# deflect-ca/banjax

Hardware: AMD Instinct MI355X
Metric: log lines/sec matched+rate-limited (node) at 1k rules; HBM GB/s vs peak (higher is better)
Workload: dtype u8

## Files before the change

banjax_amd/csrc/bjx_common.h:

```cpp
#pragma once
#include <stdint.h>

#ifdef __HIPCC__
#define BJX_HD __host__ __device__ __forceinline__
#define BJX_HDN __host__ __device__ inline
#else
#define BJX_HD inline
#define BJX_HDN inline
#endif

namespace bjx {


BJX_HD int32_t decode_rune_hd(const uint8_t *s, uint64_t n, int *width) {
  uint8_t b0 = s[0];
  if (b0 < 0x80) { *width = 1; return b0; }
  int need; uint8_t lo = 0x80, hi = 0xBF; int32_t r;
  if (b0 >= 0xC2 && b0 <= 0xDF) { need = 1; r = b0 & 0x1F; }
  else if (b0 == 0xE0) { need = 2; lo = 0xA0; r = b0 & 0x0F; }
  else if ((b0 >= 0xE1 && b0 <= 0xEC) || b0 == 0xEE || b0 == 0xEF) { need = 2; r = b0 & 0x0F; }
  else if (b0 == 0xED) { need = 2; hi = 0x9F; r = b0 & 0x0F; }
  else if (b0 == 0xF0) { need = 3; lo = 0x90; r = b0 & 0x07; }
  else if (b0 >= 0xF1 && b0 <= 0xF3) { need = 3; r = b0 & 0x07; }
  else if (b0 == 0xF4) { need = 3; hi = 0x8F; r = b0 & 0x07; }
  else { *width = 1; return 0xFFFD; }
  if (n < (uint64_t)need + 1 || s[1] < lo || s[1] > hi) { *width = 1; return 0xFFFD; }
  r = (r << 6) | (s[1] & 0x3F);
  for (int k = 2; k <= need; ++k) {
    if (s[k] < 0x80 || s[k] > 0xBF) { *width = 1; return 0xFFFD; }
    r = (r << 6) | (s[k] & 0x3F);
  }
  *width = need + 1;
  return r;
}


BJX_HD uint64_t mix64(uint64_t x) {
  x ^= x >> 33; x *= 0xff51afd7ed558ccdULL;
  x ^= x >> 33; x *= 0xc4ceb9fe1a85ec53ULL;
  x ^= x >> 33;
  return x;
}
inline uint32_t ld4(const uint8_t *p) {
  uint32_t v;
  __builtin_memcpy(&v, p, 4);
  return v;
}
#ifdef __HIPCC__
__device__ __forceinline__ uint32_t ld4(const uint8_t *p) {
  const uint32_t sh = (uint32_t)(reinterpret_cast<uintptr_t>(p) & 3);
  const uint32_t *w = reinterpret_cast<const uint32_t *>(p - sh);
  return sh ? __builtin_amdgcn_alignbyte(w[1], w[0], sh) : w[0];
}
#endif

BJX_HD uint32_t rotl32(uint32_t x, int r) { return (x << r) | (x >> (32 - r)); }

BJX_HD uint64_t hash_finish(uint32_t a, uint32_t b, uint32_t t);

BJX_HD uint64_t hash_bytes(const uint8_t *p, uint32_t n) {
  uint32_t a = 0x9E3779B9u ^ n, b = 0x7F4A7C15u + n * 0x85EBCA6Bu;
  uint32_t i = 0;
  for (; i + 4 <= n; i += 4) {
    const uint32_t w = ld4(p + i);
    a = rotl32(a ^ w, 7) * 0x27D4EB2Du;
    b = rotl32(b + w, 13) * 0x165667B1u;
  }
  uint32_t t = 0;
  for (uint32_t k = 0; i + k < n; ++k) t |= (uint32_t)p[i + k] << (8 * k);
  return hash_finish(a, b, t);
}

BJX_HD uint32_t host_fold_word(uint32_t w, uint32_t k) {
  const uint32_t r = (7u * k + 3u) & 31u;
  return (w << r) | (w >> ((32u - r) & 31u));
}
BJX_HD uint32_t host_fold_finish(uint32_t a, uint32_t n) {
  a ^= n * 0x9E3779B9u;
  a ^= a >> 15; a *= 0x2C1B3C6Du; a ^= a >> 12; a *= 0x297A2D39u; a ^= a >> 15;
  return a | 1u;
}
BJX_HD uint32_t host_fold(const uint8_t *p, uint32_t n) {
  uint32_t a = 0, k = 0, i = 0;
  for (; i + 4 <= n; i += 4, ++k) a ^= host_fold_word(ld4(p + i), k);
  if (i < n) {
    uint32_t t = 0;
    for (uint32_t b = 0; i + b < n; ++b) t |= (uint32_t)p[i + b] << (8 * b);
    a ^= host_fold_word(t, k);
  }
  return host_fold_finish(a, n);
}

BJX_HD uint64_t hash_finish(uint32_t a, uint32_t b, uint32_t t) {
  a = rotl32(a ^ t ^ 0xA5A5A5A5u, 7) * 0x27D4EB2Du;
  b = rotl32(b + t, 13) * 0x165667B1u;
  a ^= b >> 16; a *= 0x85EBCA6Bu; a ^= a >> 13; a *= 0xC2B2AE35u; a ^= a >> 16;
  b ^= a >> 15; b *= 0x2C1B3C6Du; b ^= b >> 12; b *= 0x297A2D39u; b ^= b >> 15;
  uint64_t h = ((uint64_t)a << 32) | b;
  if (h == 0 || h == ~0ULL) h = 0x1234567ULL;
  return h;
}


BJX_HD uint64_t search_stride(uint64_t lo, uint64_t hi, uint32_t K) { return (hi - lo + K - 1) / K; }
BJX_HD void search_narrow(uint64_t &lo, uint64_t &hi, uint64_t stride, uint32_t f, uint32_t K) {
  if (f == 0) { hi = lo; return; }
  uint64_t last = f - 1;
  if (f < K) hi = lo + (uint64_t)f * stride;
  else {
    last = (hi - 1 - lo) / stride;
    if (last > K - 1) last = K - 1;
  }
  lo += last * stride + 1;
}


BJX_HD int64_t go_sub(int64_t t, int64_t u) {
  int64_t d = (int64_t)((uint64_t)t - (uint64_t)u);
  if (((t ^ u) & (t ^ d)) < 0) return t < u ? INT64_MIN : INT64_MAX;
  return d;
}


BJX_HD bool window_past(int64_t ts, int64_t t0, int64_t interval) { return go_sub(ts, t0) > interval; }

BJX_HD bool window_step(int64_t ts, int64_t interval, int64_t limit, bool &valid, int64_t &hits, int64_t &start, uint32_t &mt) {
  if (!valid) { hits = 1; start = ts; mt = 0; valid = true; }
  else if (window_past(ts, start, interval)) { mt = 1; hits = 1; start = ts; }
  else { mt = 2; ++hits; }
  const bool ex = hits > limit;
  if (ex) hits = 0;
  return ex;
}

BJX_HD int64_t mod_pos(int64_t a, int64_t b) {
  if ((((uint64_t)a | (uint64_t)b) >> 32) == 0) return (int64_t)((uint32_t)a % (uint32_t)b);
  return a % b;
}

BJX_HD int64_t window_hits(int64_t h0, int64_t e, int64_t limit) {
  if (limit < 0) return 0;
  if (limit == INT64_MAX) return h0 + e;
  if (h0 > limit) return mod_pos(e - 1, limit + 1);
  return mod_pos(h0 + e, limit + 1);
}

BJX_HD int64_t ns_from_seconds(double f) {
  double x = f * 1e9;
  if (!(x >= -9223372036854775808.0 && x < 9223372036854775808.0)) return INT64_MIN;
  return (int64_t)x;
}


BJX_HD int lower_c(int c) { return (c >= 'A' && c <= 'Z') ? c + 32 : c; }

BJX_HD int parse_float_fast(const uint8_t *s, uint32_t n, double *out) {
  if (n == 0 || n > 40) return 1;
  uint64_t m = 0;
  int frac = -1, digits = 0;
  for (uint32_t i = 0; i < n; ++i) {
    uint8_t c = s[i];
    if (c >= '0' && c <= '9') {
      if (m != 0 || c != '0') ++digits;
      if (digits > 16) return 1;
      m = m * 10 + (c - '0');
      if (frac >= 0) ++frac;
    } else if (c == '.' && frac < 0) {
      frac = 0;
    } else {
      return 1;
    }
  }
  if (frac < 0) frac = 0;
  if (s[0] == '.' || (n == 1 && s[0] == '.')) return 1;
  if (m >= (1ULL << 53) || frac > 22) return 1;
  double p = 1.0;
  if (frac & 1) p *= 1e1;
  if (frac & 2) p *= 1e2;
  if (frac & 4) p *= 1e4;
  if (frac & 8) p *= 1e8;
  if (frac & 16) p *= 1e16;
  double f = (double)m;
  *out = frac ? f / p : f;
  return 0;
}

struct Decimal {
  uint8_t d[800];
  int nd, dp;
  bool neg, trunc;
};

BJX_HDN void dec_trim(Decimal *a) {
  while (a->nd > 0 && a->d[a->nd - 1] == 0) a->nd--;
  if (a->nd == 0) a->dp = 0;
}
BJX_HDN void dec_lshift(Decimal *a, unsigned k) {
  uint8_t tmp[824];
  int tw = 824;
  uint64_t n = 0;
  for (int r = a->nd - 1; r >= 0; --r) {
    n += (uint64_t)a->d[r] << k;
    uint64_t q = n / 10;
    tmp[--tw] = (uint8_t)(n - 10 * q);
    n = q;
  }
  while (n > 0) {
    uint64_t q = n / 10;
    tmp[--tw] = (uint8_t)(n - 10 * q);
    n = q;
  }
  int newnd = 824 - tw;
  int keep = newnd > 800 ? 800 : newnd;
  for (int i = 0; i < keep; ++i) a->d[i] = tmp[tw + i];
  for (int i = keep; i < newnd; ++i)
    if (tmp[tw + i]) a->trunc = true;
  a->dp += newnd - a->nd;
  a->nd = keep;
  dec_trim(a);
}
BJX_HDN void dec_rshift(Decimal *a, unsigned k) {
  int r = 0, w = 0;
  uint64_t n = 0;
  for (; (n >> k) == 0; ++r) {
    if (r >= a->nd) {
      if (n == 0) { a->nd = 0; return; }
      while ((n >> k) == 0) { n *= 10; ++r; }
      break;
    }
    n = n * 10 + a->d[r];
  }
  a->dp -= r - 1;
  const uint64_t mask = (1ULL << k) - 1;
  for (; r < a->nd; ++r) {
    uint64_t dig = n >> k;
    n &= mask;
    a->d[w++] = (uint8_t)dig;
    n = n * 10 + a->d[r];
  }
  while (n > 0) {
    uint64_t dig = n >> k;
    n &= mask;
    if (w < 800) a->d[w++] = (uint8_t)dig;
    else if (dig > 0) a->trunc = true;
    n = n * 10;
  }
  a->nd = w;
  dec_trim(a);
}
BJX_HDN void dec_shift(Decimal *a, int k) {
  if (a->nd == 0) return;
  if (k > 0) { while (k > 60) { dec_lshift(a, 60); k -= 60; } dec_lshift(a, (unsigned)k); }
  else if (k < 0) { while (k < -60) { dec_rshift(a, 60); k += 60; } dec_rshift(a, (unsigned)-k); }
}
BJX_HDN bool dec_round_up(const Decimal *a, int nd) {
  if (a->d[nd] == 5 && nd + 1 == a->nd) {
    if (a->trunc) return true;
    return nd > 0 && (a->d[nd - 1] % 2) != 0;
  }
  return a->d[nd] >= 5;
}
BJX_HDN uint64_t dec_rounded_integer(const Decimal *a) {
  if (a->dp > 20) return ~0ULL;
  int i = 0;
  uint64_t n = 0;
  for (; i < a->dp && i < a->nd; ++i) n = n * 10 + a->d[i];
  for (; i < a->dp; ++i) n *= 10;
  if (a->dp >= 0 && a->dp < a->nd && dec_round_up(a, a->dp)) ++n;
  return n;
}
BJX_HDN uint64_t dec_float_bits(Decimal *a, bool *overflow) {
  const int mantbits = 52, expbits = 11, bias = -1023;
  const int powtab[9] = {1, 3, 6, 9, 13, 16, 19, 23, 26};
  int exp = 0;
  uint64_t mant = 0;
  *overflow = false;
  if (a->nd == 0) { mant = 0; exp = bias; goto out; }
  if (a->dp > 310) goto ovf;
  if (a->dp < -330) { mant = 0; exp = bias; goto out; }
  while (a->dp > 0) {
    int n = a->dp >= 9 ? 27 : powtab[a->dp];
    dec_shift(a, -n);
    exp += n;
  }
  while (a->dp < 0 || (a->dp == 0 && a->d[0] < 5)) {
    int n = -a->dp >= 9 ? 27 : powtab[-a->dp];
    dec_shift(a, n);
    exp -= n;
  }
  exp--;
  if (exp < bias + 1) {
    int n = bias + 1 - exp;
    dec_shift(a, -n);
    exp += n;
  }
  if (exp - bias >= (1 << expbits) - 1) goto ovf;
  dec_shift(a, 1 + mantbits);
  mant = dec_rounded_integer(a);
// ... 280 lines not shown
```

banjax_amd/csrc/engine.hip:

```cpp
#include <hip/hip_runtime.h>
#include <hipcub/hipcub.hpp>

#include <algorithm>
#include <array>
#include <atomic>
#include <cstdio>
#include <cstdlib>
#include <cstring>
#include <map>
#include <tuple>
#include <memory>
#include <mutex>
#include <stdexcept>
#include <string>
#include <unordered_map>
#include <thread>
#include <vector>

#include "../../include/banjax_gpu.h"
#include "bjx_common.h"
#include "engine_types.h"
#include "regex_compiler.h"
#include "bans.h"

// ... 3072 lines not shown
      continue;
    }
    R v = s_rec[b];
    for (uint32_t u = b; u < e; ++u) {
      R nx;
      if (u + 1 < e) nx = s_rec[u + 1];
      s_out[u] = apply_step(v, tbase, rules, pr, interval, limit, valid, hits, start);
      v = nx;
    }
    st[q].hits = hits;
    st[q].start = start;
    st[q].valid = 1;
  }
  __syncthreads();
  const uint32_t s_lo = nh ? s_head[0] : n, s_hi = nh && s_cont ? s_head[nh - 1] : n;
  for (uint32_t i = s_lo + tid; i < s_hi; i += kBlock) {
    out_sorted[u0 + i] = s_out[i];
    if (wcnt) atomicAdd(&wcnt[u0 + i], 1u);
  }
}

constexpr int kBucketBits = 16;
constexpr uint32_t kBucketItems = 16;
constexpr uint32_t kBucketCap = kBlock * kBucketItems;
constexpr uint32_t kWaveRun = 8;

__global__ __launch_bounds__(kBlock) void k_bucket_bounds(uint64_t n_ev, const uint32_t *__restrict__ key, uint32_t L,
                                                          uint32_t nb, uint32_t *__restrict__ bstart) {
  const uint64_t i0 = ((uint64_t)blockIdx.x * blockDim.x + threadIdx.x) * 4;
  uint32_t k[4] = {0, 0, 0, 0};
  if (i0 + 4 <= n_ev) {
    const uint4 v = *reinterpret_cast<const uint4 *>(key + i0);
    k[0] = v.x; k[1] = v.y; k[2] = v.z; k[3] = v.w;
  } else {
    for (uint32_t j = 0; j < 4; ++j)
      if (i0 + j < n_ev) k[j] = key[i0 + j];
  }
  uint32_t prev = __shfl_up(k[3], 1);
  if ((threadIdx.x & 63) == 0 && i0 && i0 <= n_ev) prev = key[i0 - 1];
#pragma unroll
  for (uint32_t j = 0; j < 4; ++j) {
    const uint64_t i = i0 + j;
    if (i > n_ev) return;
    const uint32_t b = i < n_ev ? k[j] >> L : nb;
    const uint32_t lo = i ? (prev >> L) + 1 : 0u;
    for (uint32_t x = lo; x <= b; ++x) bstart[x] = (uint32_t)i;
    prev = k[j];
  }
}


template <typename R>
__device__ __forceinline__ void wave_chunk(uint32_t u0, uint32_t p, const R &rv, uint32_t na, bool first, int64_t tbase,
                                           const DevRule *__restrict__ rules, uint32_t &r0, int64_t &I, int64_t &Lim,
                                           bool &valid, int64_t &hits, int64_t &start, uint8_t *s_out,
                                           uint32_t *__restrict__ wcnt) {
  const uint32_t lane = threadIdx.x & 63;
  const bool act = lane < na;
  const uint32_t r = rv.rule_id();
  const int64_t ts = rv.time(tbase);
  if (first) {
    r0 = __shfl(r, 0);
    I = rules[r0].interval_ns;
    Lim = rules[r0].hits;
  }
  bool same = true;
  if (r != r0) same = rules[r].interval_ns == I && rules[r].hits == Lim;
  uint32_t mt = BJX_INSIDE_INTERVAL;
  bool ex = false;
  if (__ballot(!same) == 0) {
    int32_t a = valid ? -1 : 0;
    int64_t Tw = valid ? start : __shfl(ts, 0);
    uint32_t wa = 0, wmt = valid ? BJX_INSIDE_INTERVAL : BJX_FIRST_TIME;
    int64_t wh0 = valid ? hits : 0;
    for (;;) {
      const unsigned long long m = __ballot(act && (int32_t)lane > a && window_past(ts, Tw, I));
      if (!m) break;
      a = __ffsll(m) - 1;
      Tw = __shfl(ts, a);
      if ((int32_t)lane >= a) { wa = (uint32_t)a; wh0 = 0; wmt = BJX_OUTSIDE_INTERVAL; }
    }
    const int64_t hh = window_hits(wh0, (int64_t)(lane - wa) + 1, Lim);
    ex = hh == 0;
    if (lane == wa) mt = wmt;
    hits = __shfl(hh, (int)na - 1);
    start = Tw;
    valid = true;
  } else {
    uint32_t pr = 0xFFFFFFFFu;
    int64_t iv = 0, lm = 0;
    for (uint32_t i = 0; i < na; ++i) {
      const uint8_t o = apply_event(__shfl(r, (int)i), true, __shfl(ts, (int)i), rules, pr, iv, lm, valid, hits, start);
      if (lane == i) { mt = (o >> 1) & 3u; ex = (o & 8) != 0; }
    }
  }
  if (act) {
    s_out[p] = outcome_byte(rv.seen(), mt, ex);
    if (wcnt) atomicAdd(&wcnt[u0 + p], 1u);
  }
}

template <typename R>
__device__ __forceinline__ void bucket_wave_runs(const R *__restrict__ rec, uint32_t u0, uint32_t n, uint32_t nh, uint32_t nwv,
                                                 const uint16_t *s_ord_top, const uint16_t *s_head, const uint16_t *s_lk,
                                                 const uint16_t *s_perm, uint8_t *s_out, uint32_t qb, int64_t tbase,
                                                 const DevRule *__restrict__ rules, StSlot *__restrict__ st,
                                                 uint32_t *__restrict__ wcnt) {
  const uint32_t lane = threadIdx.x & 63;
  uint32_t t = threadIdx.x >> 6;
  if (t >= nwv) return;
  uint32_t b, e, q;
  auto run_at = [&](uint32_t tt, uint32_t &bb, uint32_t &ee, uint32_t &qq) {
    const uint32_t h = *(s_ord_top - tt);
    bb = s_head[h];
    ee = h + 1 < nh ? s_head[h + 1] : n;
    qq = qb | s_lk[bb];
  };
  auto pos_at = [&](uint32_t cc, uint32_t ee) { return (uint32_t)s_perm[cc + (lane < ee - cc ? lane : 0u)]; };
  run_at(t, b, e, q);
  uint32_t c = b;
  StSlot nslot = st[q];
  uint32_t np = pos_at(c, e);
  R nrv = rec[u0 + np];
  bool valid = false;
  int64_t hits = 0, start = 0, I = 0, Lim = 0;
  uint32_t r0 = 0;
  for (;;) {
    const uint32_t p = np, na = min(64u, e - c);
    const R rv = nrv;
    const bool first = c == b, last = c + 64 >= e;
    if (first) { valid = nslot.valid != 0; hits = nslot.hits; start = nslot.start; }
    uint32_t t2 = t, b2 = b, e2 = e, q2 = q, c2 = c + 64;
    if (last) {
      t2 = t + kBlock / 64;
      if (t2 < nwv) { run_at(t2, b2, e2, q2); c2 = b2; }
    }
    const bool more = t2 < nwv;
    if (more) {
      if (last) nslot = st[q2];
      np = pos_at(c2, e2);
      nrv = rec[u0 + np];
    }
    wave_chunk(u0, p, rv, na, first, tbase, rules, r0, I, Lim, valid, hits, start, s_out, wcnt);
    if (last && lane == 0) {
      st[q].hits = hits;
      st[q].start = start;
      st[q].valid = 1;
    }
    if (!more) break;
    t = t2; b = b2; e = e2; q = q2; c = c2;
  }
}

#ifdef BJX_BK_STOP
#define BJX_BK_STAGE(k)                                                           \
  if (BJX_BK_STOP == (k)) {                                                       \
    for (uint32_t i = tid; i < n; i += kBlock) out_sorted[u0 + i] = s_out[i];     \
    return;                                                                       \
  }
#define BJX_BK_LANE_RUNS (BJX_BK_STOP == 3 ? nfront : nh - nwv)
#else
#define BJX_BK_STAGE(k)
#define BJX_BK_LANE_RUNS (nh - nwv)
#endif
#ifdef BJX_BK_CENSUS
__device__ unsigned long long g_bk_census[8];
#endif

template <typename R>
__global__ __launch_bounds__(kBlock) void k_bucket_apply(const uint32_t *__restrict__ key, const R *__restrict__ rec,
                                                         const uint32_t *__restrict__ bstart, uint32_t L, int64_t tbase,
                                                         const DevRule *__restrict__ rules, StSlot *__restrict__ st,
                                                         uint8_t *__restrict__ out_sorted, uint32_t *__restrict__ big,
                                                         unsigned long long *__restrict__ n_big, uint32_t *__restrict__ wcnt,
                                                         uint32_t wave_min) {
  using Sort = hipcub::BlockRadixSort<uint32_t, kBlock, kBucketItems>;
  static_assert(kBucketCap <= 4096, "positions ride in 12 key bits");
  constexpr uint32_t kLongRun = 8;
  __shared__ union {
    typename Sort::TempStorage sort;
    uint32_t lk[kBucketCap];
    uint16_t ho[2 * kBucketCap];
  } s_u;
  __shared__ uint16_t s_lk[kBucketCap];
  __shared__ uint16_t s_perm[kBucketCap];
  uint16_t *const s_head = s_u.ho;
  uint16_t *const s_ord = s_u.ho + kBucketCap;
  __shared__ uint8_t s_out[kBucketCap];
  __shared__ uint32_t s_wsum[kBlock / 64], s_front, s_back, s_nwave;
  const uint32_t tid = threadIdx.x, lane = tid & 63, wave = tid >> 6;
  const uint32_t bk = blockIdx.x, u0 = bstart[bk], n = bstart[bk + 1] - u0;
  if (n == 0) return;
  if (n > kBucketCap) {
    if (tid == 0) big[atomicAdd(n_big, 1ull)] = bk;
    return;
  }
  const uint32_t mask = (1u << L) - 1u;
  for (uint32_t i = tid; i < n; i += kBlock) s_u.lk[i] = key[u0 + i] & mask;
#ifdef BJX_BK_STOP
  for (uint32_t i = tid; i < n; i += kBlock) s_out[i] = outcome_byte(true, BJX_INSIDE_INTERVAL, false);
#endif
  if (tid == 0) { s_front = 0; s_back = 0; s_nwave = 0; }
  __syncthreads();
  uint32_t k[kBucketItems];
#pragma unroll
  for (uint32_t j = 0; j < kBucketItems; ++j) {
    const uint32_t i = tid * kBucketItems + j;
    k[j] = ((i < n ? s_u.lk[i] : mask) << 12) | i;
  }
  __syncthreads();
  Sort(s_u.sort).SortBlockedToStriped(k, 12, 12 + (int)L);
  __syncthreads();
#pragma unroll
  for (uint32_t j = 0; j < kBucketItems; ++j) {
    const uint32_t r = j * kBlock + tid;
    s_lk[r] = (uint16_t)(k[j] >> 12);
    s_perm[r] = (uint16_t)(k[j] & 0xFFFu);
  }
  __syncthreads();
  BJX_BK_STAGE(1)
  uint32_t fl = 0;
#pragma unroll
  for (uint32_t j = 0; j < kBucketItems; ++j) {
    const uint32_t i = tid * kBucketItems + j;
    if (i < n && (i == 0 || s_lk[i] != s_lk[i - 1])) fl |= 1u << j;
  }
  const uint32_t cnt = __popc(fl);
  uint32_t x = cnt;
#pragma unroll
  for (int d = 1; d < 64; d <<= 1) {
    const uint32_t y = __shfl_up(x, d);
    if (lane >= (uint32_t)d) x += y;
  }
  if (lane == 63) s_wsum[wave] = x;
  __syncthreads();
  uint32_t base = x - cnt, nh = 0;
  for (uint32_t w = 0; w < kBlock / 64; ++w) {
    if (w < wave) base += s_wsum[w];
    nh += s_wsum[w];
  }
  for (uint32_t j = 0; fl; ++j, fl >>= 1)
    if (fl & 1) s_head[base++] = (uint16_t)(tid * kBucketItems + j);
  __syncthreads();
  for (uint32_t h = tid; h < nh; h += kBlock) {
    const uint32_t len = (h + 1 < nh ? s_head[h + 1] : n) - s_head[h];
    if (len >= wave_min) s_ord[kBucketCap - 1 - atomicAdd(&s_nwave, 1u)] = (uint16_t)h;
    else if (len >= kLongRun) s_ord[atomicAdd(&s_front, 1u)] = (uint16_t)h;
    else s_ord[nh - 1 - atomicAdd(&s_back, 1u)] = (uint16_t)h;
#ifdef BJX_BK_CENSUS
    atomicAdd(&g_bk_census[0], (unsigned long long)len);
    atomicAdd(&g_bk_census[1], 1ull);
    for (uint32_t c = 0; c < 3; ++c)
      if (len >= (8u << c * (c + 1) / 2)) {
        atomicAdd(&g_bk_census[2 + 2 * c], (unsigned long long)len);
        atomicAdd(&g_bk_census[3 + 2 * c], 1ull);
      }
#endif
  }
  __syncthreads();
  BJX_BK_STAGE(2)
  const uint32_t qb = bk << L;
  const uint32_t nwv = s_nwave, nfront = s_front;
  bucket_wave_runs(rec, u0, n, nh, nwv, s_ord + kBucketCap - 1, s_head, s_lk, s_perm, s_out, qb, tbase, rules, st, wcnt);
  for (uint32_t t = tid; t < BJX_BK_LANE_RUNS; t += kBlock) {
    const uint32_t h = s_ord[t < nfront ? t : t + nwv];
    const uint32_t b = s_head[h], e = h + 1 < nh ? s_head[h + 1] : n;
    const uint32_t q = qb | s_lk[b];
    const StSlot cur = st[q];
    bool valid = cur.valid != 0;
    int64_t hits = cur.hits, start = cur.start, interval = 0, limit = 0;
    uint32_t pr = 0xFFFFFFFFu;
    uint32_t p = s_perm[b];
    R rv = rec[u0 + p];
    for (uint32_t u = b; u < e; ++u) {
      R nx;
      uint32_t pn = 0;
      if (u + 1 < e) { pn = s_perm[u + 1]; nx = rec[u0 + pn]; }
      s_out[p] = apply_step(rv, tbase, rules, pr, interval, limit, valid, hits, start);
      if (wcnt) atomicAdd(&wcnt[u0 + p], 1u);
      rv = nx;
      p = pn;
    }
    st[q].hits = hits;
    st[q].start = start;
    st[q].valid = 1;
  }
  __syncthreads();
  for (uint32_t i = tid; i < n; i += kBlock) out_sorted[u0 + i] = s_out[i];
}

__global__ __launch_bounds__(kBlock) void k_big_gather(const uint4 *__restrict__ seg, uint32_t n_seg, uint64_t total,
                                                       const uint32_t *__restrict__ key, uint32_t *__restrict__ ko,
                                                       uint32_t *__restrict__ po) {
  const uint64_t i = (uint64_t)blockIdx.x * blockDim.x + threadIdx.x;
  if (i >= total) return;
  uint32_t lo = 0, hi = n_seg - 1;
  while (lo < hi) {
    const uint32_t mid = (lo + hi + 1) >> 1;
    if (seg[mid].z <= i) lo = mid;
    else hi = mid - 1;
  }
  const uint4 s = seg[lo];
  const uint32_t src = s.x + (uint32_t)(i - s.z);
  ko[i] = key[src];
  po[i] = src;
}

template <typename R>
__global__ __launch_bounds__(kBlock) void k_big_recs(uint64_t n, const uint32_t *__restrict__ pos, const R *__restrict__ rec,
                                                     R *__restrict__ out) {
  const uint64_t i = (uint64_t)blockIdx.x * blockDim.x + threadIdx.x;
  if (i < n) out[i] = rec[pos[i]];
}

__global__ __launch_bounds__(kBlock) void k_big_outs(uint64_t n, const uint32_t *__restrict__ pos, const uint8_t *__restrict__ o,
                                                     uint8_t *__restrict__ out_sorted, const uint32_t *__restrict__ wsrc,
                                                     uint32_t *__restrict__ wcnt) {
  const uint64_t i = (uint64_t)blockIdx.x * blockDim.x + threadIdx.x;
  if (i >= n) return;
  out_sorted[pos[i]] = o[i];
  if (wcnt) atomicAdd(&wcnt[pos[i]], wsrc[i]);
}

__device__ __forceinline__ uint32_t block_min_u32(uint32_t v, uint32_t *s_red) {
  for (int o = 32; o > 0; o >>= 1) v = min(v, (uint32_t)__shfl_xor((int)v, o));
  __syncthreads();
  if ((threadIdx.x & 63) == 0) s_red[threadIdx.x >> 6] = v;
  __syncthreads();
  uint32_t m = s_red[0];
  for (uint32_t w = 1; w < kBlock / 64; ++w) m = min(m, s_red[w]);
  return m;
}

template <typename P>
__device__ uint64_t block_first(uint64_t lo, uint64_t hi, P pred, uint32_t *s_red) {
  while (lo < hi) {
    const uint64_t stride = search_stride(lo, hi, kBlock);
    const uint64_t p = lo + (uint64_t)threadIdx.x * stride;
    const bool ok = p < hi && pred(p);
    const uint32_t f = block_min_u32(ok ? threadIdx.x : (uint32_t)kBlock, s_red);
    search_narrow(lo, hi, stride, f, kBlock);
  }
  return hi;
}

constexpr uint64_t kLongSerial = 512;

struct LongRuns {
  const uint64_t *head;
  uint64_t *end;
  uint64_t *off;
  int64_t *t0;
  int64_t *h0;
  uint32_t *flags;
  uint64_t *win;
  uint32_t *nwin;
  uint64_t n;
  uint32_t *wcnt;
};

template <typename Rec>
__global__ __launch_bounds__(kBlock) void k_long_ends(uint64_t n_ev, const uint32_t *__restrict__ key,
                                                      const Rec *__restrict__ rec, int64_t base, const StSlot *__restrict__ st,
                                                      const DevRule *__restrict__ rules, LongRuns R, uint64_t *__restrict__ len) {
  __shared__ uint32_t s_red[kBlock / 64];
  const uint64_t r = blockIdx.x;
  const uint64_t head = R.head[r];
  const uint32_t q = key[head];
  const uint64_t end = block_first(head + 1, n_ev, [&](uint64_t i) { return key[i] != q; }, s_red);
  if (threadIdx.x != 0) return;
  R.end[r] = end;
  len[r] = end - head;
// ... 4355 lines not shown
    if (kept_ips > n_ips || kept_bytes > used || kept_st > e->st_cap)
      throw BjxError(BJX_ERR_DEVICE, "internal: expiry counts exceed the tables");

    const uint64_t ip_cap = std::min(e->ip_cap, std::max(e->ip_cap0, next_pow2(kept_ips * 4 / 3 + 1024)));
    const uint64_t st_cap = std::min(e->st_cap, std::max(e->st_cap0, next_pow2(kept_st * 4 / 3 + 1024)));
    const uint64_t arena_cap = std::min(S.arena_cap, std::max(e->arena_cap0, next_pow2(2 * kept_bytes + 4096)));
    ExpAlloc nw;
    IpSlot *n_ip = nw.get<IpSlot>(ip_cap);
    uint32_t *n_first = nw.get<uint32_t>(ip_cap);
    uint64_t *n_off = nw.get<uint64_t>(ip_cap);
    uint32_t *n_len = nw.get<uint32_t>(ip_cap);
    uint32_t *n_ipst = nw.get<uint32_t>(ip_cap);
    uint8_t *n_arena = nw.get<uint8_t>(arena_cap);
    StSlot *n_stt = nw.get<StSlot>(st_cap);
    if (nw.nomem) throw BjxError(BJX_ERR_NOMEM, "bjx_state_expire: no device memory for the new tables (state unchanged)");
    HIP_OK(hipEventRecord(ev[2], st));
    HIP_OK(hipMemsetAsync(n_ip, 0, ip_cap * sizeof(IpSlot), st));
    HIP_OK(hipMemsetAsync(n_first, 0xFF, ip_cap * 4, st));
    HIP_OK(hipMemsetAsync(n_ipst, 0xFF, ip_cap * 4, st));
    HIP_OK(hipMemsetAsync(n_stt, 0, st_cap * sizeof(StSlot), st));
    if (n_ips) {
      hipLaunchKernelGGL(k_exp_arena, dim3(grid_for(n_ips)), dim3(kBlock), 0, st, n_ips, keep, nid, noff, S.ip_off, S.ip_len,
                         S.arena, used, n_arena, arena_cap, n_off, n_len);
      HIP_OK(hipGetLastError());
    }
    hipLaunchKernelGGL(k_exp_st, dim3(grid_for(e->st_cap)), dim3(kBlock), 0, st, e->st_cap, S.st, cutoff_ns, n_ips, nid, n_stt,
                       st_cap - 1);
    HIP_OK(hipGetLastError());
    hipLaunchKernelGGL(k_exp_ip, dim3(grid_for(e->ip_cap)), dim3(kBlock), 0, st, e->ip_cap, S.ip, n_ips, keep, nid, n_ip,
                       ip_cap - 1);
    HIP_OK(hipGetLastError());
    HIP_OK(hipEventRecord(ev[3], st));
    HIP_OK(hipStreamSynchronize(st));

    nw.take();
    for (void *p : {(void *)S.ip, (void *)S.ip_first, (void *)S.ip_off, (void *)S.ip_len, (void *)S.ip_st, (void *)S.arena,
                    (void *)S.st})
      (void)hipFree(p);
    S.ip = n_ip; S.ip_first = n_first; S.ip_off = n_off; S.ip_len = n_len; S.ip_st = n_ipst; S.arena = n_arena; S.st = n_stt;
    S.ip_mask = ip_cap - 1;
    S.st_mask = st_cap - 1;
    S.arena_cap = arena_cap;
    S.ip_st_cap = ip_cap;
    if (st_cap > (1ull << 32)) S.hot_name = kNone;
    else if (e->st_cap > (1ull << 32)) e->bound_uid = 0;
    e->ip_cap = ip_cap;
    e->st_cap = st_cap;
    e->sort2_hold = 0;
    hipLaunchKernelGGL(k_exp_counters, dim3(1), dim3(64), 0, st, S.counters, kept_ips, kept_bytes, (uint64_t)kept_st);
    HIP_OK(hipGetLastError());
    HIP_OK(hipStreamSynchronize(st));
    e->host_counters[0] = kept_ips; e->host_counters[1] = kept_bytes; e->host_counters[2] = kept_st;
    e->counters_fresh = false;
    if (out) {
      float a = 0, b = 0;
      HIP_OK(hipEventElapsedTime(&a, ev[0], ev[1]));
      HIP_OK(hipEventElapsedTime(&b, ev[2], ev[3]));
      out->states_before = n_st; out->states_dropped = n_st - std::min<uint64_t>(n_st, kept_st);
      out->ips_before = n_ips; out->ips_dropped = n_ips - kept_ips;
      out->arena_bytes_before = used; out->arena_bytes_after = kept_bytes;
      out->device_bytes_before = bytes_before;
      out->device_bytes_after = state_device_bytes(ip_cap, st_cap, arena_cap);
      out->device_ms = (double)a + (double)b;
    }
    return BJX_OK;
  } catch (const BjxError &x) {
    e->last_error = x.what();
    return x.code;
  } catch (const std::bad_alloc &) {
    e->last_error = "host out of memory";
    return BJX_ERR_NOMEM;
  }
}

extern "C" size_t bjx_state_dump(bjx_engine *e, char *out, size_t cap) {
  if (!e) return 0;
  std::lock_guard<std::mutex> g(e->mu);
  try {
    HIP_OK(hipSetDevice(e->device));
    read_counters(e);
    const uint64_t n_ips = e->host_counters[0], used = e->host_counters[1];
    std::vector<uint64_t> off(n_ips);
    std::vector<uint32_t> len(n_ips);
    std::vector<StSlot> st(e->st_cap);
    std::vector<uint8_t> arena(used);
    HIP_OK(hipMemcpy(off.data(), e->S.ip_off, n_ips * 8, hipMemcpyDeviceToHost));
    HIP_OK(hipMemcpy(len.data(), e->S.ip_len, n_ips * 4, hipMemcpyDeviceToHost));
    HIP_OK(hipMemcpy(arena.data(), e->S.arena, used, hipMemcpyDeviceToHost));
    HIP_OK(hipMemcpy(st.data(), e->S.st, e->st_cap * sizeof(StSlot), hipMemcpyDeviceToHost));
    std::vector<std::vector<std::pair<uint32_t, uint64_t>>> per_ip(n_ips);
    for (uint64_t i = 0; i < e->st_cap; ++i)
      if (st[i].key && st[i].valid) per_ip[(st[i].key >> 24) - 1].push_back({(uint32_t)(st[i].key & 0xFFFFFF), i});
    std::string s;
    char buf[96];
    for (uint64_t id = 0; id < n_ips; ++id) {
      s.append(reinterpret_cast<const char *>(arena.data() + off[id]), len[id]);
      s += ":\n";
      std::sort(per_ip[id].begin(), per_ip[id].end(),
                [&](const std::pair<uint32_t, uint64_t> &a, const std::pair<uint32_t, uint64_t> &b) {
                  return e->names[a.first] < e->names[b.first];
                });
      for (auto &p : per_ip[id]) {
        s += "\t" + e->names[p.first] + ":\n";
        snprintf(buf, sizeof buf, "\t\t{%lld %lld}\n", (long long)st[p.second].hits, (long long)st[p.second].start);
        s += buf;
      }
      s += "\n";
    }
    if (out && cap) memcpy(out, s.data(), std::min(cap, s.size()));
    return s.size();
  } catch (const BjxError &x) {
    e->last_error = x.what();
    return 0;
  }
}

#include "../../include/banjax_gpu_debug.h"

extern "C" int bjx_debug_rule_match_host(const bjx_ruleset *rs, size_t i, const uint8_t *text, size_t n) {
  if (!rs || i >= rs->rules.size() || (n && !text)) return BJX_ERR_ARG;
  return dfa_match_host(rs->rules[i].rx, text, n) ? 1 : 0;
}
extern "C" int bjx_debug_set_dfa_state_cap(uint32_t cap) {
  set_dfa_state_cap(cap);
  std::lock_guard<std::mutex> g(g_rx_mu);
  g_rx_cache.clear();
  return BJX_OK;
}
extern "C" int bjx_debug_force_wide_nfa(int on) {
  set_force_wide_nfa(on != 0);
  std::lock_guard<std::mutex> g(g_rx_mu);
  g_rx_cache.clear();
  return BJX_OK;
}
extern "C" int bjx_debug_set_ip_hash_mask(bjx_engine *e, uint64_t mask) {
  if (!e) return BJX_ERR_ARG;
  std::lock_guard<std::mutex> g(e->mu);
  e->dbg_hash_mask = mask;
  return BJX_OK;
}
extern "C" int bjx_debug_set_claim_budget(bjx_engine *e, uint64_t max_new) {
  if (!e) return BJX_ERR_ARG;
  std::lock_guard<std::mutex> g(e->mu);
  e->dbg_budget = max_new;
  return BJX_OK;
}
extern "C" int bjx_debug_set_slot_cache(bjx_engine *e, int on) {
  if (!e) return BJX_ERR_ARG;
  std::lock_guard<std::mutex> g(e->mu);
  e->dbg_slot_cache = on < 0 ? -1 : on != 0;
  e->bound_uid = 0;
  return BJX_OK;
}
extern "C" size_t bjx_debug_phase_ms(bjx_engine *e, double *out, size_t cap) {
  if (!e) return 0;
  for (size_t k = 0; k < cap && k < (size_t)bjx_engine::kPhases; ++k) out[k] = e->phase_ms[k];
  if (cap > (size_t)bjx_engine::kPhases) out[bjx_engine::kPhases] = e->exchange_ms;
  return bjx_engine::kPhases + 1;
}
extern "C" size_t bjx_debug_kernel_ms(bjx_engine *e, double *out, size_t cap) {
  if (!e) return 0;
  const double v[5] = {e->kernel_ms[0], e->kernel_ms[1], e->kernel_ms[2], (double)e->last_line_kernel,
                       e->last_line_kernel == 2 ? (double)kL2Win : e->last_line_kernel == 1 ? (double)kSpanBytes : 0.0};
  for (size_t k = 0; k < cap && k < 5; ++k) out[k] = v[k];
  return 5;
}
extern "C" size_t bjx_debug_scan_stats(bjx_engine *e, uint64_t *out, size_t cap) {
  if (!e) return 0;
  std::lock_guard<std::mutex> g(e->mu);
  if (e->S.counters) read_counters(e);
  const uint64_t v[12] = {e->scan_stats[0], e->scan_stats[1], e->scan_stats[2], e->scan_stats[3], e->scan_stats[4],
                          e->ip_cap, e->host_counters[0], e->st_cap, e->host_counters[2], e->scan_stats[5],
                          e->last_grouping, e->last_long_runs};
  for (size_t k = 0; k < 12 && k < cap; ++k) out[k] = v[k];
  return 12;
}
extern "C" int bjx_debug_rule_lead(const bjx_ruleset *rs, size_t i) {
  if (!rs || i >= rs->rules.size()) return BJX_ERR_ARG;
  const auto &rx = rs->rules[i].rx;
  return rx.mode == kModePrefilter && rx.pref_lead ? (int)rx.lead_dist : -1;
}

extern "C" size_t bjx_debug_rule_literal(const bjx_ruleset *rs, size_t i, char *out, size_t cap) {
  if (!rs || i >= rs->rules.size()) return 0;
  const CompiledRegex &rx = rs->rules[i].rx;
  std::string l = std::to_string((int)rx.mode) + " " + std::to_string((int)rx.pref_equivalent);
  for (const PrefLit &pl : rx.pref) {
    l += "\n" + std::to_string(pl.gram_off) + " ";
    for (char c : pl.ci) l += c ? '1' : '0';
    l += " " + pl.s;
  }
  for (const PrefLit &pl : rx.anchor) {
    l += std::string("\n^") + (rx.anchor_equivalent ? "=" : "~") + " ";
    for (char c : pl.ci) l += c ? '1' : '0';
    l += " " + pl.s;
  }
  if (out && cap) memcpy(out, l.data(), std::min(cap, l.size()));
  return l.size();
}
```

include/banjax_gpu_debug.h:

```cpp
#ifndef BANJAX_GPU_DEBUG_H
#define BANJAX_GPU_DEBUG_H
#include <stddef.h>
#include <stdint.h>
#include "banjax_gpu.h"
#ifdef __cplusplus
extern "C" {
#endif
int bjx_debug_rule_match_host(const bjx_ruleset *rs, size_t rule_idx, const uint8_t *text, size_t n);
size_t bjx_debug_rule_literal(const bjx_ruleset *rs, size_t rule_idx, char *out, size_t cap);
int bjx_debug_rule_lead(const bjx_ruleset *rs, size_t rule_idx);
int bjx_debug_regex_parse(const char *pattern, size_t len, char *err, size_t err_len);
size_t bjx_debug_phase_ms(bjx_engine *e, double *out, size_t cap);
size_t bjx_debug_kernel_ms(bjx_engine *e, double *out, size_t cap);
size_t bjx_debug_scan_stats(bjx_engine *e, uint64_t *out, size_t cap);
int bjx_debug_set_ip_hash_mask(bjx_engine *e, uint64_t mask);
int bjx_debug_set_claim_budget(bjx_engine *e, uint64_t max_new);
int bjx_debug_set_slot_cache(bjx_engine *e, int on);
int bjx_debug_set_dfa_state_cap(uint32_t cap);
int bjx_debug_force_wide_nfa(int on);
#ifdef __cplusplus
}
#endif
#endif
```

Measured before the change: 2.585 billion.

## Replace hipcub block radix sort in bucket apply with custom wave-ballot ranking

Swaps the hipcub BlockRadixSort in k_bucket_apply for a custom one- or two-pass counting rank. Each pass uses wave ballots and mbcnt to find matching digits, packed 16-bit per-wave histograms with atomics, and a block scan. Keys are read straight from global memory instead of being staged in shared memory first. This should cut sort passes and shared-memory footprint, and an occupancy hint of 4 blocks is added to launch bounds. A debug entry point exposes the ranker for testing, and the ordering must stay stable to match the old sort.

```diff
diff --git a/banjax_amd/csrc/bjx_common.h b/banjax_amd/csrc/bjx_common.h
--- a/banjax_amd/csrc/bjx_common.h
+++ b/banjax_amd/csrc/bjx_common.h
@@ -144,6 +144,23 @@
   if (h0 > limit) return mod_pos(e - 1, limit + 1);
   return mod_pos(h0 + e, limit + 1);
 }
+
+constexpr uint32_t kRankWaves = 4;
+constexpr uint32_t kRankPassBits = 8;
+constexpr uint32_t kRankWaveChunks = 16;
+
+BJX_HD uint32_t rank_passes(uint32_t L) { return L <= kRankPassBits ? 1u : 2u; }
+BJX_HD uint32_t rank_pass_bits(uint32_t L, uint32_t p) {
+  if (L <= kRankPassBits) return L;
+  return p == 0 ? (L + 1) / 2 : L / 2;
+}
+BJX_HD uint32_t rank_pass_shift(uint32_t L, uint32_t p) { return p == 0 ? 0u : rank_pass_bits(L, 0); }
+BJX_HD void rank_wave_chunks(uint32_t n, uint32_t v, uint32_t &c0, uint32_t &c1) {
+  const uint32_t C = (n + 63) / 64, per = (C + kRankWaves - 1) / kRankWaves;
+  c0 = v * per < C ? v * per : C;
+  c1 = c0 + per < C ? c0 + per : C;
+}
+BJX_HD uint32_t rank_scan_index(uint32_t d, uint32_t v) { return d * kRankWaves + v; }
 
 BJX_HD int64_t ns_from_seconds(double f) {
   double x = f * 1e9;
diff --git a/banjax_amd/csrc/engine.hip b/banjax_amd/csrc/engine.hip
--- a/banjax_amd/csrc/engine.hip
+++ b/banjax_amd/csrc/engine.hip
@@ -3248,6 +3248,110 @@
   }
 }
 
+static_assert(kBlock / 64 == (int)kRankWaves && kBlock >= (1 << kRankPassBits), "one thread per digit, four waves");
+static_assert(kBucketCap == 64 * kRankWaves * kRankWaveChunks, "a wave's chunks fit its registers");
+__device__ __forceinline__ void bucket_rank(const uint32_t *__restrict__ key, uint32_t n, uint32_t L, uint32_t *s_pass,
+                                            uint16_t *s_hist, uint32_t *s_wsum, uint16_t *s_lk, uint16_t *s_perm) {
+  const uint32_t tid = threadIdx.x, lane = tid & 63;
+  const uint32_t wave = (uint32_t)__builtin_amdgcn_readfirstlane((int)(tid >> 6));
+  const uint32_t mask = (1u << L) - 1u, np = rank_passes(L);
+  uint2 *const s_hist4 = reinterpret_cast<uint2 *>(s_hist);
+  uint32_t *const s_hist2 = reinterpret_cast<uint32_t *>(s_hist);
+  uint32_t c0, c1;
+  rank_wave_chunks(n, wave, c0, c1);
+  const uint32_t first = c0 * 64 + lane, nw = c1 - c0;
+  const uint32_t m = first < n ? min(nw, (n - first + 63) >> 6) : 0u;
+  const uint32_t hsh = (wave & 1u) * 16u;
+#pragma unroll
+  for (uint32_t p = 0; p < 2; ++p) {
+    if (p >= np) break;
+    const uint32_t w = rank_pass_bits(L, p), sh = 12 + rank_pass_shift(L, p), dm = (1u << w) - 1u;
+    uint32_t it[kRankWaveChunks], pr[kRankWaveChunks] = {};
+    if (p == 0) {
+#pragma unroll
+      for (uint32_t j = 0; j < kRankWaveChunks; ++j) {
+        const uint32_t raw = key[min(first + j * 64, n - 1)] & mask;
+        it[j] = (raw << 12) | (first + j * 64) | (j < m ? 0u : ~0u);
+      }
+    } else {
+#pragma unroll
+      for (uint32_t j = 0; j < kRankWaveChunks; ++j) {
+        const uint32_t raw = s_pass[min(first + j * 64, n - 1)];
+        it[j] = raw | (j < m ? 0u : ~0u);
+      }
+    }
+    if (tid <= dm) s_hist4[tid] = make_uint2(0u, 0u);
+    __syncthreads();
+    for (uint32_t j = 0; j < kRankWaveChunks; ++j) {
+      if (j >= nw) break;
+      {
+        const uint32_t d = (it[j] >> sh) & dm;
+        const bool act = (int32_t)it[j] >= 0;
+        const unsigned long long actm = __ballot(act);
+        uint32_t o_lo = ~(uint32_t)actm, o_hi = ~(uint32_t)(actm >> 32);
+        for (uint32_t b = 0; b < w; ++b) {
+          const uint32_t mine = (uint32_t)((int32_t)(d << (31u - b)) >> 31);
+          const unsigned long long bal = __ballot(mine != 0u);
+          o_lo |= (uint32_t)bal ^ mine;
+          o_hi |= (uint32_t)(bal >> 32) ^ mine;
+        }
+        const uint32_t p_lo = ~o_lo, p_hi = ~o_hi;
+        const uint32_t lrank = __builtin_amdgcn_mbcnt_hi(p_hi, __builtin_amdgcn_mbcnt_lo(p_lo, 0u));
+        uint32_t old = 0;
+        if (act && lrank == 0)
+          old = atomicAdd(&s_hist2[rank_scan_index(d, wave) >> 1], (uint32_t)(__popc(p_lo) + __popc(p_hi)) << hsh);
+        const uint32_t leader = min((uint32_t)__ffs(p_lo) - 1u, (uint32_t)__ffs(p_hi) + 31u);
+        old = (uint32_t)__builtin_amdgcn_ds_bpermute((int)(leader << 2), (int)old);
+        pr[j] = ((old >> hsh) & 0xFFFFu) + lrank;
+      }
+    }
+    __syncthreads();
+    uint32_t h0 = 0, h1 = 0, h2 = 0, h3 = 0;
+    if (tid <= dm) {
+      const uint2 v = s_hist4[tid];
+      h0 = v.x & 0xFFFFu; h1 = v.x >> 16; h2 = v.y & 0xFFFFu; h3 = v.y >> 16;
+    }
+    const uint32_t tot = h0 + h1 + h2 + h3;
+    uint32_t x = tot;
+#pragma unroll
+    for (int o = 1; o < 64; o <<= 1) {
+      const uint32_t y = __shfl_up(x, o);
+      if (lane >= (uint32_t)o) x += y;
+    }
+    if (lane == 63) s_wsum[wave] = x;
+    __syncthreads();
+    uint32_t base = x - tot;
+    for (uint32_t v = 0; v < wave; ++v) base += s_wsum[v];
+    if (tid <= dm) {
+      const uint32_t e1 = base + h0, e2 = e1 + h1, e3 = e2 + h2;
+      s_hist4[tid] = make_uint2(base | e1 << 16, e2 | e3 << 16);
+    }
+    __syncthreads();
+#pragma unroll
+    for (uint32_t j = 0; j < kRankWaveChunks; ++j) {
+      const uint32_t r = s_hist[rank_scan_index((it[j] >> sh) & dm, wave)] + pr[j];
+      if ((int32_t)it[j] >= 0) {
+        if (p + 1 < np) s_pass[r] = it[j];
+        else { s_lk[r] = (uint16_t)(it[j] >> 12); s_perm[r] = (uint16_t)(it[j] & 0xFFFu); }
+      }
+    }
+    __syncthreads();
+  }
+}
+
+__global__ __launch_bounds__(kBlock, 4) void k_debug_bucket_rank(const uint32_t *__restrict__ key, uint32_t n, uint32_t L,
+                                                              uint16_t *__restrict__ lk_out, uint16_t *__restrict__ perm_out) {
+  __shared__ uint32_t s_pass[kBucketCap];
+  __shared__ uint16_t s_lk[kBucketCap], s_perm[kBucketCap];
+  __shared__ alignas(8) uint16_t s_hist[kRankWaves << kRankPassBits];
+  __shared__ uint32_t s_wsum[kBlock / 64];
+  bucket_rank(key, n, L, s_pass, s_hist, s_wsum, s_lk, s_perm);
+  for (uint32_t i = threadIdx.x; i < n; i += kBlock) {
+    lk_out[i] = s_lk[i];
+    perm_out[i] = s_perm[i];
+  }
+}
+
 #ifdef BJX_BK_STOP
 #define BJX_BK_STAGE(k)                                                           \
   if (BJX_BK_STOP == (k)) {                                                       \
@@ -3264,22 +3368,21 @@
 #endif
 
 template <typename R>
-__global__ __launch_bounds__(kBlock) void k_bucket_apply(const uint32_t *__restrict__ key, const R *__restrict__ rec,
+__global__ __launch_bounds__(kBlock, 4) void k_bucket_apply(const uint32_t *__restrict__ key, const R *__restrict__ rec,
                                                          const uint32_t *__restrict__ bstart, uint32_t L, int64_t tbase,
                                                          const DevRule *__restrict__ rules, StSlot *__restrict__ st,
                                                          uint8_t *__restrict__ out_sorted, uint32_t *__restrict__ big,
                                                          unsigned long long *__restrict__ n_big, uint32_t *__restrict__ wcnt,
                                                          uint32_t wave_min) {
-  using Sort = hipcub::BlockRadixSort<uint32_t, kBlock, kBucketItems>;
   static_assert(kBucketCap <= 4096, "positions ride in 12 key bits");
   constexpr uint32_t kLongRun = 8;
   __shared__ union {
-    typename Sort::TempStorage sort;
-    uint32_t lk[kBucketCap];
+    uint32_t pass[kBucketCap];
     uint16_t ho[2 * kBucketCap];
   } s_u;
   __shared__ uint16_t s_lk[kBucketCap];
   __shared__ uint16_t s_perm[kBucketCap];
+  __shared__ alignas(8) uint16_t s_hist[kRankWaves << kRankPassBits];
   uint16_t *const s_head = s_u.ho;
   uint16_t *const s_ord = s_u.ho + kBucketCap;
   __shared__ uint8_t s_out[kBucketCap];
@@ -3291,29 +3394,11 @@
     if (tid == 0) big[atomicAdd(n_big, 1ull)] = bk;
     return;
   }
-  const uint32_t mask = (1u << L) - 1u;
-  for (uint32_t i = tid; i < n; i += kBlock) s_u.lk[i] = key[u0 + i] & mask;
 #ifdef BJX_BK_STOP
   for (uint32_t i = tid; i < n; i += kBlock) s_out[i] = outcome_byte(true, BJX_INSIDE_INTERVAL, false);
 #endif
   if (tid == 0) { s_front = 0; s_back = 0; s_nwave = 0; }
-  __syncthreads();
-  uint32_t k[kBucketItems];
-#pragma unroll
-  for (uint32_t j = 0; j < kBucketItems; ++j) {
-    const uint32_t i = tid * kBucketItems + j;
-    k[j] = ((i < n ? s_u.lk[i] : mask) << 12) | i;
-  }
-  __syncthreads();
-  Sort(s_u.sort).SortBlockedToStriped(k, 12, 12 + (int)L);
-  __syncthreads();
-#pragma unroll
-  for (uint32_t j = 0; j < kBucketItems; ++j) {
-    const uint32_t r = j * kBlock + tid;
-    s_lk[r] = (uint16_t)(k[j] >> 12);
-    s_perm[r] = (uint16_t)(k[j] & 0xFFFu);
-  }
-  __syncthreads();
+  bucket_rank(key + u0, n, L, s_u.pass, s_hist, s_wsum, s_lk, s_perm);
   BJX_BK_STAGE(1)
   uint32_t fl = 0;
 #pragma unroll
@@ -7975,6 +8060,32 @@
   e->bound_uid = 0;
   return BJX_OK;
 }
+extern "C" int bjx_debug_bucket_rank(bjx_engine *e, const uint32_t *low_keys, uint32_t n, uint32_t L, uint16_t *lk_out,
+                                     uint16_t *perm_out) {
+  if (!e || n > kBucketCap || L < 1 || L > 15 || (n && (!low_keys || !lk_out || !perm_out))) return BJX_ERR_ARG;
+  if (n == 0) return BJX_OK;
+  std::lock_guard<std::mutex> g(e->mu);
+  DevBuf<uint32_t> keys;
+  DevBuf<uint16_t> tabs;
+  int rc = BJX_OK;
+  try {
+    HIP_OK(hipSetDevice(e->device));
+    keys.ensure(n);
+    tabs.ensure(2 * (size_t)n);
+    HIP_OK(hipMemcpyAsync(keys.p, low_keys, (size_t)n * 4, hipMemcpyHostToDevice, e->stream));
+    hipLaunchKernelGGL(k_debug_bucket_rank, dim3(1), dim3(kBlock), 0, e->stream, keys.p, n, L, tabs.p, tabs.p + n);
+    HIP_OK(hipGetLastError());
+    HIP_OK(hipMemcpyAsync(lk_out, tabs.p, (size_t)n * 2, hipMemcpyDeviceToHost, e->stream));
+    HIP_OK(hipMemcpyAsync(perm_out, tabs.p + n, (size_t)n * 2, hipMemcpyDeviceToHost, e->stream));
+    HIP_OK(hipStreamSynchronize(e->stream));
+  } catch (const BjxError &x) {
+    e->last_error = x.what();
+    rc = x.code;
+  }
+  keys.release();
+  tabs.release();
+  return rc;
+}
 extern "C" size_t bjx_debug_phase_ms(bjx_engine *e, double *out, size_t cap) {
   if (!e) return 0;
   for (size_t k = 0; k < cap && k < (size_t)bjx_engine::kPhases; ++k) out[k] = e->phase_ms[k];
diff --git a/include/banjax_gpu_debug.h b/include/banjax_gpu_debug.h
--- a/include/banjax_gpu_debug.h
+++ b/include/banjax_gpu_debug.h
@@ -18,6 +18,8 @@
 int bjx_debug_set_slot_cache(bjx_engine *e, int on);
 int bjx_debug_set_dfa_state_cap(uint32_t cap);
 int bjx_debug_force_wide_nfa(int on);
+int bjx_debug_bucket_rank(bjx_engine *e, const uint32_t *low_keys, uint32_t n, uint32_t L, uint16_t *lk_out,
+                          uint16_t *perm_out);
 #ifdef __cplusplus
 }
 #endif
```

Measured after the change: 2.582 billion. About the same (-0.1%).
